# seokjuchung/point-cloud-cnn-segmentation

Measured on AMD Instinct MI355X. Metric: M voxels/sec fwd+bwd, 128^3 grid batch=4 (points/s of the PointNet training step: forward + weighted CE + backward + Adam), higher is better.
Workload: dtype bf16; 1 GPU; PointNetSegmentation train step, 4 scenes x 128^3 points per GPU, C=2; global_batch=4, parallelism=dp1

## Files before the change

point-cloud-cnn-segmentation_amd/csrc/fused_bwd.hip:

```cpp
#include "kernel_prims.h"

namespace {

constexpr int THREADS = 512;
constexpr int COUT = 512, CIN = 64, MS = 64;
constexpr int WT_ROWB = COUT * 2;
constexpr int DY_ROWB = COUT * 2 + 32;
constexpr int X_ROWB = CIN * 2 + 32;
constexpr int OFF_DY = CIN * WT_ROWB;
constexpr int OFF_X = OFF_DY + MS * DY_ROWB;
constexpr int OFF_OUT = OFF_X + MS * X_ROWB;
constexpr int OUT_ROWB = CIN * 2 + 8;
constexpr int OFF_COEF = OFF_OUT + MS * OUT_ROWB;
constexpr int OFF_H = OFF_COEF + 3 * CIN * 4;
constexpr int H_ROWB = CIN * 2;
constexpr int LDS_BYTES = OFF_H + CIN * H_ROWB;
static_assert(LDS_BYTES <= 160 * 1024, "LDS budget");
constexpr int SLAB_F = COUT * CIN + CIN * CIN + CIN;
constexpr int DY_CPR = COUT / 8, DY_RP = THREADS / DY_CPR, DY_NCH = MS / DY_RP;
constexpr int X_CPR = CIN / 8, X_RP = THREADS / X_CPR;
static_assert(X_RP == MS, "one x chunk per thread");

PCS_DEV int wt_off(int c, int slot) { return c * WT_ROWB + ((slot ^ (c & 15)) << 4); }

// ... 514 lines not shown
  for (int u = 0; u < F::TPW_D; ++u)
#pragma unroll
    for (int r = 0; r < 4; ++r)
#pragma unroll
      for (int o = 1; o < 16; o <<= 1) {
        s1[u][r] += __shfl_xor(s1[u][r], o);
        s2[u][r] += __shfl_xor(s2[u][r], o);
      }
  float2 *red = reinterpret_cast<float2 *>(lds);
  if (l16 == 0) {
#pragma unroll
    for (int u = 0; u < F::TPW_D; ++u)
#pragma unroll
      for (int r = 0; r < 4; ++r) red[mb * CB + (cbd + u) * 16 + 4 * g + r] = make_float2(s1[u][r], s2[u][r]);
  }
  __syncthreads();
  for (int c = tid; c < CB; c += THREADS) {
    float t1 = 0.f, t2 = 0.f;
#pragma unroll
    for (int b = 0; b < F::NMB; ++b) { t1 += red[b * CB + c].x; t2 += red[b * CB + c].y; }
    *reinterpret_cast<float2 *>(a.stats + ((int64_t)chunk * CIN + n0 + c) * 2) =
        make_float2(t1, a.erstd[n0 + c] * (t2 - a.emean[n0 + c] * t1));
  }
}

template <int COUT, int CIN, int CB, int MS>
int launch_bn(const pcs_gemm_args &a, float *wpart, int64_t rps, hipStream_t s) {
  const int nb = (int)(a.num_scenes * a.chunks_per_scene) * (CIN / CB);
  if (a.c_mask && a.addend) return pcs_set_einval("pcs_dgrad_wgrad_bn", "mask and addend together");
  if (a.c_mask)
    hipLaunchKernelGGL((dgrad_wgrad_bn_kernel<COUT, CIN, CB, MS, true, false>), dim3(nb), dim3(THREADS), 0, s, a, wpart, rps);
  else if (a.addend) {
    if constexpr (FB<COUT, CIN, CB, MS, false, true>::FITS)
      hipLaunchKernelGGL((dgrad_wgrad_bn_kernel<COUT, CIN, CB, MS, false, true>), dim3(nb), dim3(THREADS), 0, s, a, wpart,
                         rps);
    else
      return pcs_set_einval("pcs_dgrad_wgrad_bn", "no addend variant at this shape (LDS)");
  } else
    hipLaunchKernelGGL((dgrad_wgrad_bn_kernel<COUT, CIN, CB, MS, false, false>), dim3(nb), dim3(THREADS), 0, s, a,
                       wpart, rps);
  PCS_CHECK_LAUNCH();
  return 0;
}

struct BnShape { int cout, cin, cb, ms; };
constexpr BnShape kBnShapes[] = {{64, 64, 64, 64}, {128, 64, 64, 64}};

const BnShape *bn_shape(int K, int Ncols) {
  for (const BnShape &b : kBnShapes)
    if (b.cout == K && b.cin == Ncols) return &b;
  return nullptr;
}

}

extern "C" int64_t pcs_dgrad_wgrad_bn_workspace(pcs_gemm_args *a) {
  if (!a || a->num_scenes <= 0 || a->scene_rows <= 0) return pcs_set_einval("pcs_dgrad_wgrad_bn_workspace", "bad geometry");
  if (pcs_seg4_applicable(*a)) {
    pcs_seg4_geometry(a);
    return (int64_t)a->num_scenes * a->chunks_per_scene * a->K * a->Ncols * 4;
  }
  const BnShape *sh = bn_shape(a->K, a->Ncols);
  if (a->dtype != PCS_BF16 || !sh || (a->flags & PCS_FLAG_GENERIC))
    return pcs_set_einval("pcs_dgrad_wgrad_bn_workspace",
                          "bf16 with (Cout, Cin) = K x Ncols in {64x64, 128x64} only");
  const int nblk = sh->cin / sh->cb;
  const int64_t target = sh->cout == 64 ? 512 : 256;
  int64_t sps = (target + a->num_scenes * nblk - 1) / (a->num_scenes * nblk);
  const int64_t max_sps = (a->scene_rows + 4 * sh->ms - 1) / (4 * sh->ms);
  if (sps > max_sps) sps = max_sps;
  if (sps < 1) sps = 1;
  const int64_t rps = ((a->scene_rows + sps - 1) / sps + sh->ms - 1) / sh->ms * sh->ms;
  a->chunks_per_scene = (int32_t)((a->scene_rows + rps - 1) / rps);
  return (int64_t)a->num_scenes * a->chunks_per_scene * a->K * a->Ncols * 4;
}

extern "C" int pcs_dgrad_wgrad_bn(const pcs_gemm_args *ap, float *partial, float *dW, int64_t ldw,
                                  pcs_stream_t stream) {
  if (!ap || !partial || !dW) return pcs_set_einval("pcs_dgrad_wgrad_bn", "null argument");
  pcs_gemm_args a = *ap;
  if (pcs_dgrad_wgrad_bn_workspace(&a) < 0) return PCS_EINVAL;
  if (a.chunks_per_scene != ap->chunks_per_scene)
    return pcs_set_einval("pcs_dgrad_wgrad_bn", "chunks_per_scene must come from pcs_dgrad_wgrad_bn_workspace");
  if (!a.A || !a.A2 || !a.pa || !a.pb || !a.pc || !a.W || !a.C || !a.Yp || !a.es || !a.et || !a.emean ||
      !a.erstd || !a.stats)
    return pcs_set_einval("pcs_dgrad_wgrad_bn", "missing operand (A, A2, pa, pb, pc, W, C, Yp, es, et, emean, "
                                                "erstd, stats)");
  if (a.scene_rows * a.num_scenes >= (int64_t)1 << 31) return pcs_set_einval("pcs_dgrad_wgrad_bn", "M must be < 2^31");
  if (pcs_seg4_applicable(a)) {
    const int rc = pcs_seg4_launch(a, partial, reinterpret_cast<hipStream_t>(stream));
    if (rc) return rc;
    const int nslab = (int)(a.num_scenes * a.chunks_per_scene);
    return pcs_reduce_partials(partial, nslab, (int64_t)a.K * a.Ncols, 1.0f, dW, ldw ? ldw : a.Ncols, a.Ncols, stream);
  }
  const BnShape *sh = bn_shape(a.K, a.Ncols);
  const int64_t rps = ((a.scene_rows + a.chunks_per_scene - 1) / a.chunks_per_scene + sh->ms - 1) / sh->ms * sh->ms;
  hipStream_t s = reinterpret_cast<hipStream_t>(stream);
  int rc;
  if (a.K == 64) rc = launch_bn<64, 64, 64, 64>(a, partial, rps, s);
  else rc = launch_bn<128, 64, 64, 64>(a, partial, rps, s);
  if (rc) return rc;
  const int nslab = (int)(a.num_scenes * a.chunks_per_scene);
  return pcs_reduce_partials(partial, nslab, (int64_t)a.K * a.Ncols, 1.0f, dW, ldw ? ldw : a.Ncols, a.Ncols, stream);
}
```

point-cloud-cnn-segmentation_amd/engine.py:

```python
from __future__ import annotations

import ctypes as ct
from dataclasses import dataclass, field

import torch

from . import _lib as L

BN_EPS = 1e-5
MAX_INPUT_DIM = 8
MAX_CLASSES = 256
BN_MOMENTUM = 0.1
DROPOUT_P = 0.3

CONVS = [
    ("conv1", None, 64, "bn1"),
    ("conv2", 64, 64, "bn2"),
    ("conv3", 64, 64, "bn3"),
    ("conv4", 64, 128, "bn4"),
    ("conv5", 128, 1024, "bn5"),
    ("global_feat", 1024, 1024, "bn_global"),
    ("seg_conv1", 1088, 512, "bn_seg1"),
    ("seg_conv2", 512, 256, "bn_seg2"),
    ("seg_conv3", 256, 128, "bn_seg3"),
# ... 20 lines not shown


def flat_layout(num_classes: int, input_dim: int = 4):
    reg = dict(param_layout(num_classes, input_dim))
    names = [f"{bn}.{w}" for bn, _ in BNS for w in ("weight", "bias")]
    for conv in _EARLY_CONVS + ("global_feat",) + _SEG:
        names += [f"{conv}.weight", f"{conv}.bias"]
    return [(n, reg[n]) for n in names]


def flat_offsets(num_classes: int, input_dim: int = 4):
    offs, off = {}, 0
    for n, shape in flat_layout(num_classes, input_dim):
        offs[n] = off
        off += int(torch.Size(shape).numel())
    return offs, off


def bucket_ranges(num_classes: int, input_dim: int = 4):
    offs, total = flat_offsets(num_classes, input_dim)
    return {"seg": (offs["seg_conv1.weight"], total + FLAT_EXTRA),
            "global": (offs["global_feat.weight"], offs["seg_conv1.weight"]),
            "tail": (0, offs["global_feat.weight"])}


def check_dims(num_classes: int, input_dim: int):
    if not 1 <= int(input_dim) <= MAX_INPUT_DIM:
        raise ValueError(f"pcs_amd supports input_dim 1..{MAX_INPUT_DIM} (the reference's points carry "
                         f"4: x, y, z, e); got {input_dim}")
    if not 1 <= int(num_classes) <= MAX_CLASSES:
        raise ValueError(f"pcs_amd supports 1..{MAX_CLASSES} classes (seg_conv4 + CE head kernel); "
                         f"got {num_classes}")


def _dt(dtype: str):
    if dtype == "fp32":
        return L.F32, torch.float32
    if dtype in ("bf16", "fp8"):
        return L.BF16, torch.bfloat16
    raise ValueError(f"compute dtype must be 'fp32', 'bf16' or 'fp8', got {dtype!r}")


@dataclass(frozen=True)
class Paths:
    flags: int
    bf16: bool
    wide_fast: bool
    glds: bool
    fp8: bool
    fused12: bool
    trunk32: bool
    gram4_stats: bool
    draw_beside_gram: bool


def resolve_paths(dtype: str, flags: int = 0, eval_trunk: str = "fp32", fused_seg12: bool = True,
                  draw_beside_gram: bool = True, dropout_draw: str = "paired", *, train: bool, masks_given: bool) -> Paths:
    bf16 = dtype in ("bf16", "fp8")
    wide_fast = bf16 and not (flags & L.FLAG_GENERIC)
    return Paths(flags=flags, bf16=bf16, wide_fast=wide_fast, glds=wide_fast and not (flags & L.FLAG_NO_GLDS),
                 fp8=dtype == "fp8", fused12=bool(train and wide_fast and fused_seg12),
                 trunk32=not train and bf16 and eval_trunk == "fp32", gram4_stats=bool(train and bf16),
                 draw_beside_gram=bool(train and not masks_given and wide_fast and draw_beside_gram
                                       and dropout_draw != "independent"))


@dataclass
class BNCoef:
    mean: torch.Tensor
    rstd: torch.Tensor
    scale: torch.Tensor
    shift: torch.Tensor
    scene_sum: torch.Tensor

    def bnrelu(self):
        return dict(pa=self.scale, pb=self.shift)


@dataclass
class Saved:
    B: int
    N: int
    train: bool
    paths: Paths = None
    ys: dict = field(default_factory=dict)
    bn: dict = field(default_factory=dict)
    masks: tuple = (None, None)
    g: torch.Tensor = None
    am: torch.Tensor = None
    ysel: torch.Tensor = None
    x: torch.Tensor = None
    logits: torch.Tensor = None
    head: dict = None
    wc: dict = None
    gram4: tuple = None
    gram2: object = None
    a5_colsum: torch.Tensor = None
    gram5: tuple = None
    wg_eff: torch.Tensor = None
    sbias_s1: torch.Tensor = None
    mask_ready: object = None


def _f32(dev, *shape):
    return torch.empty(*shape, dtype=torch.float32, device=dev)


def _struct(cls, **members):
    a = cls()
    for k, v in members.items():
        setattr(a, k, L.ptr(v) if torch.is_tensor(v) else v)
    return a


class _Bwd:

    def __init__(self, gflat, offsets, bufA):
        self.gflat, self.offsets = gflat, offsets
        self.coefs = {}
        self.bufA = bufA
        self.bufB = None
        self.keep = []
        self.st = None
        self.keep_scale = 1.0 / (1.0 - DROPOUT_P)

    def G(self, name):
        return self.gflat[self.offsets[name]:]


class Engine:

    def __init__(self, num_classes: int, dtype: str = "fp32", input_dim: int = 4, eval_trunk: str = "fp32"):
        check_dims(num_classes, input_dim)
        if eval_trunk not in ("fp32", "bf16"):
            raise ValueError(f"eval_trunk must be 'fp32' or 'bf16', got {eval_trunk!r}")
        self.input_dim = input_dim
        self.C = num_classes
        self.dtype = dtype
        self.dt, self.tdt = _dt(dtype)
        self.fp8 = dtype == "fp8"
        self.a5_dt = L.FP8 if self.fp8 else self.dt
        self.eval_trunk = eval_trunk
        self.layout = param_layout(num_classes, input_dim)
        self.numel = {n: int(torch.Size(s).numel()) for n, s in self.layout}
        self.offsets, self.total_params = flat_offsets(num_classes, input_dim)
        self.buckets = bucket_ranges(num_classes, input_dim)
        self._geo = {}
        self._side = {}
        self.flags = 0
        self.timing = None
        self.timing_tags = None
        self.record_pool_rows = False
        self.last_pool_rows = None
        self.pool_rows_override = None
        self.capture = None
        self.perturb = None
        self.fused_seg12 = True
        self.draw_beside_gram = True
        self.dropout_draw = "paired"
        L.load()

    def _launch(self, tag, name, *args):
        if self.timing is None or tag is None or (self.timing_tags is not None and tag not in self.timing_tags):
            return L.call(name, *args)
        st, en = torch.cuda.Event(enable_timing=True), torch.cuda.Event(enable_timing=True)
        st.record()
        r = L.call(name, *args)
        en.record()
        self.timing.setdefault(tag, []).append((st, en))
        return r

    def _dims(self, sv):
        return sv.B, sv.N, sv.B * sv.N, sv.x.device, L.stream_ptr()

    def _side_stream(self, dev):
        st = self._side.get(dev)
        if st is None:
            st = self._side.setdefault(dev, torch.cuda.Stream(device=dev))
        return st

    @staticmethod
    def _gemm_args(B, N, K, ncols, dtype, pro=L.PRO_RAW, epi=L.EPI_FWD, cps=0, flags=0, **members):
        return _struct(L.GemmArgs, num_scenes=B, scene_rows=N, K=K, Ncols=ncols, dtype=dtype, prologue=pro,
                       epilogue=epi, chunks_per_scene=cps, flags=flags, **members)

    def geometry(self, B, N, K, ncols, pro=L.PRO_BNRELU, epi=L.EPI_FWD, dtype=None, flags=None):
        dtype = self.dt if dtype is None else dtype
        flags = self.flags if flags is None else flags
        key = (B, N, K, ncols, pro, epi, flags, dtype)
        if key not in self._geo:
            a = self._gemm_args(B, N, K, ncols, dtype, pro, epi, 0, flags)
            rpc = L.workspace("pcs_gemm_geometry", a)
            self._geo[key] = (a.chunks_per_scene, rpc)
        return self._geo[key]

    def _empty(self, *shape, dtype=None, device):
        return torch.empty(*shape, dtype=dtype or self.tdt, device=device)

    def cast_weights(self, P):
        dev = P["conv2.weight"].device
        wc = {}
        s = L.stream_ptr()
        for conv, cin, cout, _ in CONVS:
            if conv in ("conv1", "seg_conv4"):
                continue
            W = P[f"{conv}.weight"]
            rows, ld = W.shape[0], W.shape[1]
            cols = 64 if conv == "seg_conv1" else ld
            Wc = self._empty(rows, cols, device=dev)
            WcT = self._empty(cols, rows, device=dev)
# ... 37 lines not shown
        self._launch(tag, "pcs_gemm", a, L.stream_ptr())

    def _wgrad_args(self, sv, cout, cin, dy_mode, x_mode, dW, ldw=0, x_keep_scale=1.0, **members):
        return _struct(L.WgradArgs, num_scenes=sv.B, scene_rows=sv.N, Cout=cout, Cin=cin, dtype=self.dt, dy_mode=dy_mode,
                       x_mode=x_mode, x_keep_scale=x_keep_scale, dW=dW, ldw=ldw, flags=sv.paths.flags, **members)

    def _wgrad(self, sv, cout, cin, dy_mode, x_mode, dW, conv1=False, tag=None, **kw):
        a = self._wgrad_args(sv, cout, cin, dy_mode, x_mode, dW, **kw)
        if conv1:
            a.splits_per_scene = max(1, min((1024 + sv.B - 1) // sv.B, (sv.N + 255) // 256))
            nbytes = sv.B * a.splits_per_scene * cout * cin * 4
        else:
            nbytes = L.workspace("pcs_wgrad_workspace", a)
        ws = _f32(dW.device, max(nbytes // 4, 1))
        a.partial = ws.data_ptr()
        self._launch(tag, "pcs_conv1_wgrad" if conv1 else "pcs_wgrad", a, L.stream_ptr())
        return ws

    def _rounded(self, W):
        if self.dt == L.F32:
            return W
        out = torch.empty_like(W)
        L.call("pcs_round_weight", W, W.numel(), self.dt, out, L.stream_ptr())
        return out

    def _gram(self, Y, s_, t_, B, N, C, tag=None):
        dev = Y.device
        G, S = _f32(dev, C, C), _f32(dev, C)
        sps = ct.c_int32(0)
        nbytes = L.workspace("pcs_gram_workspace", B, N, C, self.dt, ct.byref(sps))
        ws = _f32(dev, max(nbytes // 4, 1))
        self._launch(tag, "pcs_gram", Y, s_, t_, B, N, C, self.dt, sps.value, ws, G, S, L.stream_ptr())
        return G, S, ws

    def _gram_raw(self, a5, G, beside=None):
        M = a5.shape[0]
        nbytes = L.workspace("pcs_gram_raw_workspace", M, 1024)
        ws = _f32(a5.device, nbytes // 4)
        if beside is not None:
            beside()
        self._launch("wgrad:global_feat", "pcs_gram_raw", a5, M, 1024, self.a5_dt, ws, nbytes, G, L.stream_ptr())
        return ws

    def forward(self, P, bufs, x, *, train, masks=None, seed=0, head_mode=L.HEAD_FWD,
                labels=None, class_weight=None, wsum=None, want_logits=True, saved=None):
        if not x.is_cuda:
            raise RuntimeError("pcs_amd runs on a HIP device only (no CPU fallback)")
        B, N, D = x.shape
        if D != self.input_dim:
            raise ValueError(f"expected x of shape (B, N, {self.input_dim}), got {tuple(x.shape)}")
        x = x.contiguous().float()
        sv = Saved(B=B, N=N, train=train) if saved is None else saved
        sv.B, sv.N, sv.train, sv.x = B, N, train, x
        sv.gram4 = None
        sv.paths = pt = resolve_paths(self.dtype, self.flags, self.eval_trunk, self.fused_seg12, self.draw_beside_gram,
                                      self.dropout_draw, train=train, masks_given=masks is not None)
        live = {}
        if train and masks is None and not pt.draw_beside_gram:
            self._draw_masks(sv, seed)
        sv.wc = self.cast_weights(P)
        self._trunk(P, bufs, sv)
        self._conv5(P, bufs, sv, live)
        self._global_feat(P, bufs, sv, live, seed)
        self._seg(P, bufs, sv, live, masks)
        sv.logits = _f32(x.device, B, N, self.C) if want_logits else None
        if head_mode == L.HEAD_CE:
            sv.head = self._head(P, sv, L.HEAD_CE, labels=labels, class_weight=class_weight, wsum=wsum)
        else:
            self._head(P, sv, L.HEAD_FWD)
        return sv

    def _draw_masks(self, sv, seed, max_wg=0):
        _, _, M, dev, _ = self._dims(sv)
        sv.masks = m1, m2 = tuple(torch.empty(M, w, dtype=torch.uint8, device=dev) for w in (64, 32))
        side = self._side_stream(dev)
        side.wait_stream(torch.cuda.current_stream(dev))
        with torch.cuda.stream(side):
            ss = L.stream_ptr()
            for i, (m, width) in enumerate(((m1, 512), (m2, 256))):
                if self.dropout_draw == "independent":
                    L.call("pcs_dropout_bits_independent", seed, i, M, width, DROPOUT_P, m, ss)
                else:
                    L.call("pcs_dropout_bits_bounded", seed, i, M, width, DROPOUT_P, m, max_wg, ss)
            sv.mask_ready = torch.cuda.Event()
            sv.mask_ready.record(side)
        m1.record_stream(side)
        m2.record_stream(side)

    def _stats_buf(self, sv, K, ncols):
        cps, rpc = self.geometry(sv.B, sv.N, K, ncols, flags=sv.paths.flags)
        return _f32(sv.x.device, sv.B * cps, ncols, 2), cps, rpc

    def _bridge(self, sv, conv, bn, K, split):
        _, _, M, dev, s = self._dims(sv)
        out = self._empty(M, 2 * K if split else K, device=dev)
        c = sv.bn[bn]
        L.call("pcs_bnrelu_bf16", sv.ys[conv], M, K, c.scale, c.shift, int(split), out, s)
        return out

    def _layer(self, P, bufs, sv, conv, src, offset=None, A_raw=None, K=None, **kw):
        M, dev = sv.B * sv.N, sv.x.device
        cin, ncols, bnname = _LAYERS[conv]
        K = K or cin
        st, cps, rpc = self._stats_buf(sv, K, ncols) if sv.train else (None, 0, 0)
        f32 = kw.get("dtype") == L.F32
        y = self._empty(M, ncols, device=dev, dtype=torch.float32 if f32 else None)
        W = P[f"{conv}.weight"] if f32 else sv.wc[conv][0]
        pro, A = L.PRO_RAW, A_raw
        if A_raw is None:
# ... 102 lines not shown
        sv.bn["bn_global"] = cg = self._bn_finalize(P, bufs, sv, "bn_global", live["stats"], 1024, cps_st, rpc_st,
                                                    P["global_feat.bias"])
        sv.g = _f32(dev, B, 1024)
        sv.am = torch.empty(B, 1024, dtype=torch.int32, device=dev)
        sv.ysel = _f32(dev, B, 1024)
        L.call("pcs_pool_finalize", pool, B, N, 1024, cps_g, cg.scale, cg.shift, sv.g, sv.am, sv.ysel, s)
        if self.record_pool_rows:
            self.last_pool_rows = sv.am.clone()
        if self.pool_rows_override is not None:
            sv.am.copy_(self.pool_rows_override)

    def _masks(self, sv, masks):
        _, _, M, dev, _ = self._dims(sv)
        m1 = m2 = None
        if sv.train and masks is not None:
            m1, m2 = masks
            if any(tuple(m.shape) != (M, w) or m.dtype != torch.uint8 or m.device != dev for m, w in ((m1, 64), (m2, 32))):
                raise ValueError(f"dropout masks must be uint8 [{M}, 64] and [{M}, 32] on {dev}, got "
                                 f"{tuple(m1.shape)} {m1.dtype} and {tuple(m2.shape)} {m2.dtype}")
            m1, m2 = m1.contiguous(), m2.contiguous()
        elif sv.train:
            m1, m2 = sv.masks
            torch.cuda.current_stream(dev).wait_event(sv.mask_ready)
        sv.masks = (m1, m2)
        return m1, m2, 1.0 / (1.0 - DROPOUT_P) if sv.train else 1.0

    def _seg(self, P, bufs, sv, live, masks):
        B, _, _, dev, s = self._dims(sv)
        pt = sv.paths
        sbias = _f32(dev, B, 512)
        live["soff"] = soff = _f32(dev, 512)
        Ws1 = P["seg_conv1.weight"]
        L.call("pcs_scene_gemv", sv.g, B, 1024, Ws1, Ws1.shape[1], 64, P["seg_conv1.bias"], 512, sbias, soff, s)
        sv.sbias_s1 = sbias
        if not pt.fused12:
            self._layer(P, bufs, sv, "seg_conv1", "conv2", soff, K=64, scene_bias=sbias,
                        A_raw=self._bridge(sv, "conv2", "bn2", 64, False) if pt.trunk32 else None)
        m1, m2, keep = self._masks(sv, masks)
        if pt.fused12:
            self._seg12(P, bufs, sv, sv.wc, sbias, soff, m1, keep)
        else:
            self._layer(P, bufs, sv, "seg_conv2", "seg_conv1", a_mask=m1, a_keep_scale=keep)
        self._layer(P, bufs, sv, "seg_conv3", "seg_conv2", a_mask=m2, a_keep_scale=keep)

    def _seg12(self, P, bufs, sv, wc, sbias, soff, m1, keep):
        B, N, M, dev, s = self._dims(sv)
        c2 = sv.bn["bn2"]
        rec = 64 * 64 + 64
        cps3 = sv.gram2.shape[0] // B
        per_scene = _f32(dev, B, rec)
        L.call("pcs_reduce_partials_grouped", sv.gram2, B, cps3, rec, 1.0, per_scene, s)
        tot = _f32(dev, rec)
        L.call("pcs_reduce_partials", per_scene, B, rec, 1.0, tot, 1, rec, s)
        G2 = tot[:64 * 64]
        Sb = per_scene[:, 64 * 64:].contiguous()
        Ws1 = P["seg_conv1.weight"]
        Ws1_r = self._rounded(Ws1)
        st1 = _f32(dev, B, 512, 2)
        L.call("pcs_bn_stats_gram_sbias", G2, Sb, B, N, Ws1_r, Ws1.shape[1], 64, 512, sbias, st1, s)
        sv.bn["bn_seg1"] = c1 = self._bn_finalize(P, bufs, sv, "bn_seg1", st1, 512, 1, N, soff)
        y1, y2 = self._empty(M, 512, device=dev), self._empty(M, 256, device=dev)
        a = _struct(L.Seg12Args, num_scenes=B, scene_rows=N, y2=sv.ys["conv2"], s2=c2.scale, t2=c2.shift,
                    W1=wc["seg_conv1"][0], sbias=sbias, Y1=y1, s1=c1.scale, t1=c1.shift, keep1=m1, keep_scale=keep,
                    W2=wc["seg_conv2"][0], Y2=y2)
        rpc, cps = L.workspace("pcs_fwd_seg12_geometry", a), a.chunks_per_scene
        st2 = _f32(dev, B * cps, 256, 2)
        a.stats = L.ptr(st2)
        self._launch("fwd:seg_conv1+2", "pcs_fwd_seg12", a, s)
        sv.ys["seg_conv1"], sv.ys["seg_conv2"] = y1, y2
        sv.bn["bn_seg2"] = self._bn_finalize(P, bufs, sv, "bn_seg2", st2, 256, cps, rpc, P["seg_conv2.bias"])

    def _head(self, P, sv, mode, labels=None, class_weight=None, wsum=None, dlogits=None):
        B, N, _, dev, s = self._dims(sv)
        c3 = sv.bn["bn_seg3"]
        ha = _struct(L.HeadArgs, num_scenes=B, scene_rows=N, Cin=128, num_classes=self.C, dtype=self.dt, mode=mode,
                     Y=sv.ys["seg_conv3"], s=c3.scale, t=c3.shift, W=P["seg_conv4.weight"], bias=P["seg_conv4.bias"],
                     logits=sv.logits if mode != L.HEAD_BWD else None)
        hb = None
        if mode != L.HEAD_FWD:
            L.workspace("pcs_head_geometry", ha)
            nch = B * ha.chunks_per_scene
            hb = dict(dZ=torch.empty(B * N * 1024, dtype=self.tdt, device=dev), stats=_f32(dev, nch, 128, 2),
                      wpartial=_f32(dev, nch, self.C * 129), loss_partial=_f32(dev, nch), cps=ha.chunks_per_scene,
                      nch=nch)
            ha.dZ, ha.stats = L.ptr(hb["dZ"]), L.ptr(hb["stats"])
            ha.wpartial, ha.loss_partial = L.ptr(hb["wpartial"]), L.ptr(hb["loss_partial"])
            ha.mean, ha.rstd = L.ptr(c3.mean), L.ptr(c3.rstd)
        if mode == L.HEAD_CE:
            ha.labels, ha.class_weight, ha.wsum = L.ptr(labels), L.ptr(class_weight), L.ptr(wsum)
        if mode == L.HEAD_BWD:
            dl = dlogits.reshape(B * N, self.C) if dlogits.dim() == 3 else dlogits
            if dl.dtype != torch.float32:
                dl = dl.float()
            ha.dlogits = L.ptr(dl)
            ha.dl_stride_row, ha.dl_stride_col = dl.stride(0), dl.stride(1)
            hb["dl"] = dl
        self._launch(f"head:{mode}", "pcs_head", ha, s)
        return hb

    def backward(self, P, sv, gflat, dlogits=None, on_bucket=None):
        bucket = on_bucket or (lambda name: None)
        if not sv.train:
            raise RuntimeError("backward needs a train-mode forward (BatchNorm batch statistics)")
        hb = self._head(P, sv, L.HEAD_BWD, dlogits=dlogits) if dlogits is not None else sv.head
        bw = _Bwd(gflat, self.offsets, hb["dZ"])
        scene_s1 = self._bwd_seg32(P, sv, bw, hb)
        sp = self._bwd_pool(P, sv, bw, scene_s1)
        dA2 = self._bwd_seg1_local(P, sv, bw)
        bucket("seg")
        Wg_r, st5, cps5 = self._bwd_global_dgrad(P, sv, bw, sp)
        self._bwd_global_wgrad(P, sv, bw, sp, Wg_r)
        bucket("global")
        self._bwd_conv5(P, sv, bw, st5, cps5)
        self._bwd_trunk(P, sv, bw, dA2)
        bucket("tail")
        return hb

    def _bn_bwd(self, P, sv, bw, bnname, conv, stats, cps, scene_s1=None):
        B, N, _, dev, s = self._dims(sv)
        fc = sv.bn[bnname]
        C = fc.mean.shape[0]
        al, be, ga = (_f32(dev, C) for _ in range(3))
        L.call("pcs_bn_bwd_finalize", stats, B, N, C, cps, fc.mean, fc.rstd, P[f"{bnname}.weight"], fc.scene_sum, al,
               be, ga, bw.G(f"{bnname}.weight"), bw.G(f"{bnname}.bias"), bw.G(f"{conv}.bias"), scene_s1, s)
        bw.coefs[bnname] = (al, be, ga)

    def _wgrad_bn(self, sv, bw, conv, dz, prev, x_mask=None, cin=None, ldw=0):
        al, be, ga = bw.coefs[_LAYERS[conv][2]]
        pc = sv.bn[_LAYERS[prev][2]]
        bw.keep.append(self._wgrad(
            sv, _LAYERS[conv][1], cin or _LAYERS[conv][0], L.PRO_BWD, L.PRO_BNRELU, bw.G(f"{conv}.weight"), ldw=ldw,
            tag=f"wgrad:{conv}", dZ=dz, Y=sv.ys[conv], alpha=al, beta=be, gamma=ga, X=sv.ys[prev], s=pc.scale,
            t=pc.shift, x_mask=x_mask, x_keep_scale=bw.keep_scale if x_mask is not None else 1.0))

    def _bwd_layer(self, P, sv, bw, conv, dz, prev, out, c_mask=None, addend=None, per_scene=False):
        B, N, _, dev, s = self._dims(sv)
        pt, WT = sv.paths, sv.wc[conv][1]
        cin, cout, bn = _LAYERS[conv]
        al, be, ga = bw.coefs[bn]
        pc = sv.bn[_LAYERS[prev][2]]
        f = dict(A2=sv.ys[conv], pa=al, pb=be, pc=ga, Yp=sv.ys[prev], es=pc.scale, et=pc.shift, emean=pc.mean,
                 erstd=pc.rstd, c_mask=c_mask, c_keep_scale=bw.keep_scale if c_mask is not None else 1.0, addend=addend)
        nbytes = -1
        if pt.wide_fast:
            a = self._gemm_args(B, N, cout, cin, self.dt, L.PRO_BWD, L.EPI_DGRAD, 0, pt.flags, A=dz, W=WT, C=out,
                                a_keep_scale=1.0, **f)
            nbytes = L.load().pcs_dgrad_wgrad_bn_workspace(ct.byref(a))
        if nbytes > 0:
            cps = a.chunks_per_scene
            st = _f32(dev, B * cps, cin, 2)
            ws = _f32(dev, nbytes // 4)
            a.stats = L.ptr(st)
            self._launch(f"dgrad+wgrad:{conv}", "pcs_dgrad_wgrad_bn", a, ws, bw.G(f"{conv}.weight"), 0, s)
            bw.keep.append(ws)
        else:
            cps, _ = self.geometry(B, N, cout, cin, L.PRO_BWD, L.EPI_DGRAD, flags=pt.flags)
            st = _f32(dev, B * cps, cin, 2)
            self._gemm(sv, cout, cin, L.PRO_BWD, L.EPI_DGRAD, dz, WT, out, stats=st, tag=f"dgrad:{conv}", **f)
            self._wgrad_bn(sv, bw, conv, dz, prev, x_mask=c_mask)
        bw.st = st
        scene_s1 = _f32(dev, B, pc.mean.shape[0]) if per_scene else None
        self._bn_bwd(P, sv, bw, _LAYERS[prev][2], prev, st, cps, scene_s1)
        return scene_s1

    def _bwd_seg32(self, P, sv, bw, hb):
        _, _, M, dev, s = self._dims(sv)
        m1, m2 = sv.masks
        L.call("pcs_reduce_partials", hb["wpartial"], hb["nch"], self.C * 129, 1.0, bw.G("seg_conv4.weight"),
               self.C * 129, self.C * 129, s)
        self._bn_bwd(P, sv, bw, "bn_seg3", "seg_conv3", hb["stats"], hb["cps"])
        bw.bufB = torch.empty(M * 1024, dtype=self.tdt, device=dev)
        self._bwd_layer(P, sv, bw, "seg_conv3", bw.bufA, "seg_conv2", bw.bufB, c_mask=m2)
        return self._bwd_layer(P, sv, bw, "seg_conv2", bw.bufB, "seg_conv1", bw.bufA, c_mask=m1, per_scene=True)

    def _bwd_pool(self, P, sv, bw, scene_s1):
        B, N, _, dev, s = self._dims(sv)
        a1, b1, g1 = bw.coefs["bn_seg1"]
        cg = sv.bn["bn_global"]
        bw.coefs["bn_global"] = ag, bg, gg = tuple(_f32(dev, 1024) for _ in range(3))
        sp = _f32(dev, B, 1024)
        csum = _f32(dev, B, 512)
        Ws1 = P["seg_conv1.weight"]
        pa = _struct(L.PoolBwdArgs, num_scenes=B, scene_rows=N, Cs=512, Cg=1024, col_off=64, s1_alpha=a1, s1_beta=b1,
                     s1_gamma=g1, s1_scene_s1=scene_s1, s1_scene_sum=sv.bn["bn_seg1"].scene_sum, W_s1=Ws1,
                     ldw=Ws1.shape[1], g=sv.g, ysel=sv.ysel, g_mean=cg.mean, g_rstd=cg.rstd,
                     g_gamma=P["bn_global.weight"], g_scene_sum=cg.scene_sum, dW_s1_global=bw.G("seg_conv1.weight"),
                     csum=csum, alpha=ag, beta_c=bg, gamma_c=gg, dgamma=bw.G("bn_global.weight"),
                     dbeta=bw.G("bn_global.bias"), dbias=bw.G("global_feat.bias"), sp=sp)
        L.call("pcs_pool_bwd", pa, s)
        bw.keep.append(csum)
        return sp

    def _bwd_seg1_local(self, P, sv, bw):
        B, N, M, dev, s = self._dims(sv)
        a1, b1, g1 = bw.coefs["bn_seg1"]
        dz_s1, ys, Ws1 = bw.bufA, sv.ys, P["seg_conv1.weight"]
        dA2 = torch.empty(M, 64, dtype=self.tdt, device=dev)
        if not sv.paths.wide_fast:
            self._gemm(sv, 512, 64, L.PRO_BWD, L.EPI_RAW, dz_s1, sv.wc["seg_conv1"][1], dA2,
                       A2=ys["seg_conv1"], pa=a1, pb=b1, pc=g1, tag="dgrad:seg_conv1")
            self._wgrad_bn(sv, bw, "seg_conv1", dz_s1, "conv2", cin=64, ldw=Ws1.shape[1])
            return dA2
        p2 = sv.bn["bn2"]
        Ws1_r = self._rounded(Ws1)
        WaT, Hs1 = self._empty(64, 512, device=dev), self._empty(64, 64, device=dev)
        L.call("pcs_bn_fold", Ws1_r, 512, 64, Ws1.shape[1], a1, b1, g1, self.dt, WaT, None, Hs1, s)
        fa = self._wgrad_args(sv, 512, 64, L.PRO_RAW, L.PRO_BNRELU, bw.G("seg_conv1.weight"), ldw=Ws1.shape[1],
                              dZ=dz_s1, alpha=a1, beta=b1, gamma=g1, X=ys["conv2"], s=p2.scale, t=p2.shift)
# ... 103 lines not shown
```

Baseline: 110.8 M points/s.

## Fold BN backward into conv3 dgrad/wgrad, reusing forward Gram to skip Y reread

Adds a folded-BN variant of the fused dgrad+wgrad kernel for conv3. It precomputes a folded weight WaT, a bias vector and a Gram-correction matrix H, so BN backward becomes a linear map of dZ plus the input activation X. This drops the read of the conv output Y (A2). Folded weights are split into bf16 hi/lo pairs to keep precision, at the cost of twice the MFMA work and more LDS. The weight gradient is assembled from reduced partials and the forward-pass Gram total, adding an assemble kernel and a reduction in exchange for less memory traffic.

```diff
diff --git a/point-cloud-cnn-segmentation_amd/csrc/fused_bwd.hip b/point-cloud-cnn-segmentation_amd/csrc/fused_bwd.hip
--- a/point-cloud-cnn-segmentation_amd/csrc/fused_bwd.hip
+++ b/point-cloud-cnn-segmentation_amd/csrc/fused_bwd.hip
@@ -590,10 +590,27 @@
   return nullptr;
 }
 
+int32_t bn_chunks(const pcs_gemm_args &a, const BnShape &sh, int64_t target) {
+  const int nblk = sh.cin / sh.cb;
+  int64_t sps = (target + a.num_scenes * nblk - 1) / (a.num_scenes * nblk);
+  const int64_t max_sps = (a.scene_rows + 4 * sh.ms - 1) / (4 * sh.ms);
+  if (sps > max_sps) sps = max_sps;
+  if (sps < 1) sps = 1;
+  const int64_t rps = ((a.scene_rows + sps - 1) / sps + sh.ms - 1) / sh.ms * sh.ms;
+  return (int32_t)((a.scene_rows + rps - 1) / rps);
+}
+
+bool bnf_selected(const pcs_gemm_args &a) {
+  return a.prologue == PCS_PRO_RAW && !pcs_seg4_applicable(a) && bn_shape(a.K, a.Ncols);
+}
+int64_t bnf_workspace(pcs_gemm_args *a);
+int bnf_run(const pcs_gemm_args *ap, float *workspace, float *dW, int64_t ldw, pcs_stream_t stream);
+
 }
 
 extern "C" int64_t pcs_dgrad_wgrad_bn_workspace(pcs_gemm_args *a) {
   if (!a || a->num_scenes <= 0 || a->scene_rows <= 0) return pcs_set_einval("pcs_dgrad_wgrad_bn_workspace", "bad geometry");
+  if (bnf_selected(*a)) return bnf_workspace(a);
   if (pcs_seg4_applicable(*a)) {
     pcs_seg4_geometry(a);
     return (int64_t)a->num_scenes * a->chunks_per_scene * a->K * a->Ncols * 4;
@@ -602,20 +619,14 @@
   if (a->dtype != PCS_BF16 || !sh || (a->flags & PCS_FLAG_GENERIC))
     return pcs_set_einval("pcs_dgrad_wgrad_bn_workspace",
                           "bf16 with (Cout, Cin) = K x Ncols in {64x64, 128x64} only");
-  const int nblk = sh->cin / sh->cb;
-  const int64_t target = sh->cout == 64 ? 512 : 256;
-  int64_t sps = (target + a->num_scenes * nblk - 1) / (a->num_scenes * nblk);
-  const int64_t max_sps = (a->scene_rows + 4 * sh->ms - 1) / (4 * sh->ms);
-  if (sps > max_sps) sps = max_sps;
-  if (sps < 1) sps = 1;
-  const int64_t rps = ((a->scene_rows + sps - 1) / sps + sh->ms - 1) / sh->ms * sh->ms;
-  a->chunks_per_scene = (int32_t)((a->scene_rows + rps - 1) / rps);
+  a->chunks_per_scene = bn_chunks(*a, *sh, sh->cout == 64 ? 512 : 256);
   return (int64_t)a->num_scenes * a->chunks_per_scene * a->K * a->Ncols * 4;
 }
 
 extern "C" int pcs_dgrad_wgrad_bn(const pcs_gemm_args *ap, float *partial, float *dW, int64_t ldw,
                                   pcs_stream_t stream) {
   if (!ap || !partial || !dW) return pcs_set_einval("pcs_dgrad_wgrad_bn", "null argument");
+  if (bnf_selected(*ap)) return bnf_run(ap, partial, dW, ldw, stream);
   pcs_gemm_args a = *ap;
   if (pcs_dgrad_wgrad_bn_workspace(&a) < 0) return PCS_EINVAL;
   if (a.chunks_per_scene != ap->chunks_per_scene)
@@ -641,3 +652,374 @@
   const int nslab = (int)(a.num_scenes * a.chunks_per_scene);
   return pcs_reduce_partials(partial, nslab, (int64_t)a.K * a.Ncols, 1.0f, dW, ldw ? ldw : a.Ncols, a.Ncols, stream);
 }
+
+namespace {
+
+template <int COUT, bool ADD> struct FF {
+  static constexpr int CIN = 64, MS = 64;
+  static constexpr int WT_ROWB = COUT * 2, WSW = COUT >= 128 ? 15 : 7;
+  static constexpr int DY_ROWB = COUT * 2 + 32, X_ROWB = CIN * 2 + 32;
+  static constexpr int YP_ROWB = CIN * 2 + 16, OUT_ROWB = CIN * 2 + 8, H_ROWB = CIN * 2;
+  static constexpr int OFF_DY = CIN * WT_ROWB;
+  static constexpr int OFF_X = OFF_DY + MS * DY_ROWB;
+  static constexpr int OFF_YP = OFF_X + MS * X_ROWB;
+  static constexpr int OFF_AD = OFF_YP + MS * YP_ROWB;
+  static constexpr int OFF_OUT = OFF_AD + (ADD ? MS * YP_ROWB : 0);
+  static constexpr int OFF_COEF = OFF_OUT + MS * OUT_ROWB;
+  static constexpr int OFF_H = OFF_COEF + 3 * CIN * 4;
+  static constexpr int OFF_HL = OFF_H + CIN * H_ROWB;
+  static constexpr int OFF_WL = OFF_HL + CIN * H_ROWB;
+  static constexpr int BYTES = OFF_WL + CIN * WT_ROWB;
+  static constexpr int CBW = COUT / 32;
+  static constexpr int NCH_D = MS * COUT / 8 / THREADS;
+  static_assert(MS * CIN / 8 == THREADS, "one Yp chunk per thread");
+  static_assert(4 * CIN * 8 <= OFF_DY, "end-of-pass S1 / S2 reduction area");
+};
+
+constexpr int bnf_slab(int cout, bool withg = true) { return cout * 64 + (withg ? 64 * 64 + 64 : 0); }
+
+template <int COUT, bool ADD, bool WITHG>
+__global__ __launch_bounds__(THREADS) __attribute__((amdgpu_waves_per_eu(COUT == 64 ? 4 : 1, 8))) void dgrad_wgrad_bnf_kernel(
+    pcs_gemm_args a, float *__restrict__ wpart, int64_t rows_per_split) {
+  typedef FF<COUT, ADD> F;
+  constexpr int CIN = F::CIN, MS = F::MS;
+  static_assert((COUT == 64 ? 2 : 1) * F::BYTES <= 160 * 1024, "LDS budget");
+  __shared__ __attribute__((aligned(16))) char lds[F::BYTES];
+  const int tid = threadIdx.x, lane = tid & 63, wid = tid >> 6;
+  const int chunk = xcd_remap(blockIdx.x, gridDim.x);
+  const int sps = a.chunks_per_scene;
+  const int scene = chunk / sps, sis = chunk % sps;
+  const int64_t N = a.scene_rows;
+  const int64_t lo = (int64_t)sis * rows_per_split;
+  const int64_t hi = pcs_min64(lo + rows_per_split, N);
+  const int64_t sbase = (int64_t)scene * N;
+  const bf16_t *__restrict__ dZ = reinterpret_cast<const bf16_t *>(a.A);
+  const bf16_t *__restrict__ Ypg = reinterpret_cast<const bf16_t *>(a.Yp);
+  const bf16_t *__restrict__ Adg = reinterpret_cast<const bf16_t *>(a.addend);
+  const float *__restrict__ Wt = reinterpret_cast<const float *>(a.W);
+  const float *__restrict__ Hg = reinterpret_cast<const float *>(a.W2);
+  bf16_t *__restrict__ Cg = reinterpret_cast<bf16_t *>(a.C);
+
+  auto split_to_lds = [&](const float *src, char *hi_dst, char *lo_dst) {
+    float v[8], h[8];
+    *reinterpret_cast<float4 *>(v) = *reinterpret_cast<const float4 *>(src);
+    *reinterpret_cast<float4 *>(v + 4) = *reinterpret_cast<const float4 *>(src + 4);
+    const u32x4 hi = pack_chunk(v);
+    unpack_chunk(hi, h);
+#pragma unroll
+    for (int e = 0; e < 8; ++e) v[e] -= h[e];
+    *reinterpret_cast<u32x4 *>(hi_dst) = hi;
+    *reinterpret_cast<u32x4 *>(lo_dst) = pack_chunk(v);
+  };
+  for (int i = tid; i < CIN * COUT / 8; i += THREADS) {
+    const int c = i / (COUT / 8), slot = i % (COUT / 8);
+    const int off = c * F::WT_ROWB + ((slot ^ (c & F::WSW)) << 4);
+    split_to_lds(Wt + (int64_t)c * COUT + slot * 8, lds + off, lds + F::OFF_WL + off);
+  }
+  {
+    const int c = tid / (CIN / 8), slot = tid % (CIN / 8);
+    const int off = c * F::H_ROWB + ((slot ^ (c & 7)) << 4);
+    split_to_lds(Hg + (int64_t)c * CIN + slot * 8, lds + F::OFF_H + off, lds + F::OFF_HL + off);
+  }
+  float *cf = reinterpret_cast<float *>(lds + F::OFF_COEF);
+  if (tid < CIN) { cf[tid] = a.es[tid]; cf[CIN + tid] = a.et[tid]; cf[2 * CIN + tid] = a.bias[tid]; }
+  __syncthreads();
+
+  const int pr = tid / (CIN / 8), pc = tid % (CIN / 8);
+  u32x4 rz[F::NCH_D], rp, rd;
+  auto load_step = [&](int64_t m0) {
+#pragma unroll
+    for (int i = 0; i < F::NCH_D; ++i) {
+      const int q = tid + THREADS * i, rl = q / (COUT / 8), cc = q % (COUT / 8);
+      rz[i] = *reinterpret_cast<const u32x4 *>(dZ + (sbase + pcs_min64(m0 + rl, hi - 1)) * COUT + cc * 8);
+    }
+    const int64_t off = (sbase + pcs_min64(m0 + pr, hi - 1)) * CIN + pc * 8;
+    rp = *reinterpret_cast<const u32x4 *>(Ypg + off);
+    if constexpr (ADD) rd = *reinterpret_cast<const u32x4 *>(Adg + off);
+  };
+  auto store_step = [&](int64_t m0) {
+#pragma unroll
+    for (int i = 0; i < F::NCH_D; ++i) {
+      const int q = tid + THREADS * i, rl = q / (COUT / 8), cc = q % (COUT / 8);
+      const u32x4 out = m0 + rl >= hi ? mk_u32x4(0, 0, 0, 0) : rz[i];
+      *reinterpret_cast<u32x4 *>(lds + F::OFF_DY + prow(rl) * F::DY_ROWB + cc * 16) = out;
+    }
+    float s8[8], t8[8], v[8];
+    lds_vec8(cf + pc * 8, s8); lds_vec8(cf + CIN + pc * 8, t8);
+    unpack_chunk(rp, v);
+#pragma unroll
+    for (int e = 0; e < 8; ++e) v[e] = relu(fmaf(v[e], s8[e], t8[e]));
+    u32x4 out = pack_chunk(v);
+    if (m0 + pr >= hi) out = mk_u32x4(0, 0, 0, 0);
+    *reinterpret_cast<u32x4 *>(lds + F::OFF_X + prow(pr) * F::X_ROWB + pc * 16) = out;
+    *reinterpret_cast<u32x4 *>(lds + F::OFF_YP + pr * F::YP_ROWB + pc * 16) = rp;
+    if constexpr (ADD) *reinterpret_cast<u32x4 *>(lds + F::OFF_AD + pr * F::YP_ROWB + pc * 16) = rd;
+  };
+
+  f32x4 accw[F::CBW];
+#pragma unroll
+  for (int u = 0; u < F::CBW; ++u) accw[u] = f32x4{0.f, 0.f, 0.f, 0.f};
+  f32x4 accg[2] = {f32x4{0.f, 0.f, 0.f, 0.f}, f32x4{0.f, 0.f, 0.f, 0.f}};
+  float xs = 0.f;
+  float s1[2][4], s2[2][4];
+#pragma unroll
+  for (int u = 0; u < 2; ++u)
+#pragma unroll
+    for (int r = 0; r < 4; ++r) { s1[u][r] = 0.f; s2[u][r] = 0.f; }
+
+  const int nsteps = (int)((hi - lo + MS - 1) / MS);
+  if (nsteps > 0) {
+    load_step(lo);
+    store_step(lo);
+    __builtin_amdgcn_sched_barrier(0);
+    load_step(lo + MS);
+  }
+  __syncthreads();
+
+  const int g = lane >> 4, l16 = lane & 15;
+  const int mb = wid >> 1, cbd = 2 * (wid & 1);
+  const int ob0 = wid * F::CBW / 4, cbw = wid * F::CBW % 4;
+  const char *tDY = lds + F::OFF_DY, *tX = lds + F::OFF_X;
+  const int ml = mb * 16 + l16;
+  constexpr bool ROOMY = COUT != 64;
+  auto h_frag = [&](int off_img, int kk, int u) {
+    const int c = (cbd + u) * 16 + l16;
+    return *reinterpret_cast<const bf16x8 *>(lds + off_img + c * F::H_ROWB + (((4 * kk + g) ^ (c & 7)) << 4));
+  };
+  bf16x8 hreg[ROOMY ? 2 : 1][2][2];
+  if constexpr (ROOMY) {
+#pragma unroll
+    for (int kk = 0; kk < 2; ++kk)
+#pragma unroll
+      for (int u = 0; u < 2; ++u) { hreg[0][kk][u] = h_frag(F::OFF_H, kk, u); hreg[1][kk][u] = h_frag(F::OFF_HL, kk, u); }
+  }
+  for (int st = 0; st < nsteps; ++st) {
+    const int64_t m0 = lo + (int64_t)st * MS;
+    f32x4 accd[2];
+#pragma unroll
+    for (int u = 0; u < 2; ++u) accd[u] = *reinterpret_cast<const f32x4 *>(cf + 2 * CIN + (cbd + u) * 16 + 4 * g);
+    if constexpr (ROOMY) {
+      f32x4 accl[2] = {f32x4{0.f, 0.f, 0.f, 0.f}, f32x4{0.f, 0.f, 0.f, 0.f}};
+#pragma unroll
+      for (int kk = 0; kk < COUT / 32; ++kk) {
+        const int slot = 4 * kk + g;
+        const bf16x8 yf = *reinterpret_cast<const bf16x8 *>(tDY + prow(ml) * F::DY_ROWB + slot * 16);
+#pragma unroll
+        for (int u = 0; u < 2; ++u) {
+          const int c = (cbd + u) * 16 + l16;
+          const int off = c * F::WT_ROWB + ((slot ^ (c & F::WSW)) << 4);
+          const bf16x8 wf = *reinterpret_cast<const bf16x8 *>(lds + off);
+          const bf16x8 wl = *reinterpret_cast<const bf16x8 *>(lds + F::OFF_WL + off);
+          accd[u] = __builtin_amdgcn_mfma_f32_16x16x32_bf16(wf, yf, accd[u], 0, 0, 0);
+          accl[u] = __builtin_amdgcn_mfma_f32_16x16x32_bf16(wl, yf, accl[u], 0, 0, 0);
+        }
+      }
+#pragma unroll
+      for (int kk = 0; kk < CIN / 32; ++kk) {
+        const bf16x8 xf = *reinterpret_cast<const bf16x8 *>(tX + prow(ml) * F::X_ROWB + (4 * kk + g) * 16);
+#pragma unroll
+        for (int u = 0; u < 2; ++u) {
+          accd[u] = __builtin_amdgcn_mfma_f32_16x16x32_bf16(hreg[0][kk][u], xf, accd[u], 0, 0, 0);
+          accl[u] = __builtin_amdgcn_mfma_f32_16x16x32_bf16(hreg[1][kk][u], xf, accl[u], 0, 0, 0);
+        }
+      }
+#pragma unroll
+      for (int u = 0; u < 2; ++u) accd[u] += accl[u];
+    } else {
+#pragma unroll
+      for (int kk = 0; kk < COUT / 32; ++kk) {
+        const int slot = 4 * kk + g;
+        const bf16x8 yf = *reinterpret_cast<const bf16x8 *>(tDY + prow(ml) * F::DY_ROWB + slot * 16);
+#pragma unroll
+        for (int u = 0; u < 2; ++u) {
+          const int c = (cbd + u) * 16 + l16;
+          const int off = c * F::WT_ROWB + ((slot ^ (c & F::WSW)) << 4);
+          const bf16x8 wf = *reinterpret_cast<const bf16x8 *>(lds + off);
+          const bf16x8 wl = *reinterpret_cast<const bf16x8 *>(lds + F::OFF_WL + off);
+          accd[u] = __builtin_amdgcn_mfma_f32_16x16x32_bf16(wf, yf, accd[u], 0, 0, 0);
+          accd[u] = __builtin_amdgcn_mfma_f32_16x16x32_bf16(wl, yf, accd[u], 0, 0, 0);
+        }
+      }
+#pragma unroll
+      for (int kk = 0; kk < CIN / 32; ++kk) {
+        const int slot = 4 * kk + g;
+        const bf16x8 xf = *reinterpret_cast<const bf16x8 *>(tX + prow(ml) * F::X_ROWB + slot * 16);
+#pragma unroll
+        for (int u = 0; u < 2; ++u) {
+          const int c = (cbd + u) * 16 + l16;
+          const int off = c * F::H_ROWB + ((slot ^ (c & 7)) << 4);
+          const bf16x8 hf = *reinterpret_cast<const bf16x8 *>(lds + F::OFF_H + off);
+          const bf16x8 hl = *reinterpret_cast<const bf16x8 *>(lds + F::OFF_HL + off);
+          accd[u] = __builtin_amdgcn_mfma_f32_16x16x32_bf16(hf, xf, accd[u], 0, 0, 0);
+          accd[u] = __builtin_amdgcn_mfma_f32_16x16x32_bf16(hl, xf, accd[u], 0, 0, 0);
+        }
+      }
+    }
+#pragma unroll
+    for (int kk = 0; kk < MS / 32; ++kk) {
+      const int q = (lane >> 2) & 3, p = lane & 3;
+      const int r0 = prow(32 * kk + 8 * g + q), r1 = prow(32 * kk + 8 * g + 4 + q);
+      const bf16x8 yf = tr_read(tDY, r0, r1, F::DY_ROWB, ob0 * 16 + 4 * p);
+      bf16x8 xi;
+      if constexpr (WITHG) {
+        xi = tr_read(tX, r0, r1, F::X_ROWB, mb * 16 + 4 * p);
+        const u32x4 xu = __builtin_bit_cast(u32x4, xi);
+        xs += ((bf_lo(xu.x) + bf_hi(xu.x)) + (bf_lo(xu.y) + bf_hi(xu.y))) +
+              ((bf_lo(xu.z) + bf_hi(xu.z)) + (bf_lo(xu.w) + bf_hi(xu.w)));
+      }
+#pragma unroll
+      for (int u = 0; u < F::CBW; ++u) {
+        const bf16x8 xf = tr_read(tX, r0, r1, F::X_ROWB, (cbw + u) * 16 + 4 * p);
+        accw[u] = __builtin_amdgcn_mfma_f32_16x16x32_bf16(xf, yf, accw[u], 0, 0, 0);
+        if constexpr (F::CBW == 2 && WITHG) accg[u] = __builtin_amdgcn_mfma_f32_16x16x32_bf16(xf, xi, accg[u], 0, 0, 0);
+      }
+      if constexpr (F::CBW != 2 && WITHG) {
+#pragma unroll
+        for (int u = 0; u < 2; ++u) {
+          const bf16x8 xj = tr_read(tX, r0, r1, F::X_ROWB, (cbd + u) * 16 + 4 * p);
+          accg[u] = __builtin_amdgcn_mfma_f32_16x16x32_bf16(xj, xi, accg[u], 0, 0, 0);
+        }
+      }
+    }
+    const bool live = m0 + ml < hi;
+#pragma unroll
+    for (int u = 0; u < 2; ++u) {
+      const int c = (cbd + u) * 16 + 4 * g;
+      const uint2 yp = *reinterpret_cast<const uint2 *>(lds + F::OFF_YP + ml * F::YP_ROWB + c * 2);
+      const float y[4] = {bf_lo(yp.x), bf_hi(yp.x), bf_lo(yp.y), bf_hi(yp.y)};
+      float v[4] = {accd[u][0], accd[u][1], accd[u][2], accd[u][3]};
+      if constexpr (ADD) {
+        const uint2 ad = *reinterpret_cast<const uint2 *>(lds + F::OFF_AD + ml * F::YP_ROWB + c * 2);
+        v[0] += bf_lo(ad.x); v[1] += bf_hi(ad.x); v[2] += bf_lo(ad.y); v[3] += bf_hi(ad.y);
+      }
+#pragma unroll
+      for (int r = 0; r < 4; ++r) {
+        const float dz = (live && fmaf(y[r], cf[c + r], cf[CIN + c + r]) > 0.f) ? v[r] : 0.f;
+        v[r] = dz;
+        s1[u][r] += dz;
+        s2[u][r] = fmaf(dz, y[r], s2[u][r]);
+      }
+      *reinterpret_cast<uint2 *>(lds + F::OFF_OUT + ml * F::OUT_ROWB + c * 2) =
+          make_uint2(pack2bf(v[0], v[1]), pack2bf(v[2], v[3]));
+    }
+    lds_barrier();
+    if (m0 + pr < hi)
+      st16(Cg + (sbase + m0 + pr) * CIN + pc * 8,
+           *reinterpret_cast<const u32x4 *>(lds + F::OFF_OUT + pr * F::OUT_ROWB + pc * 16));
+    if (st + 1 < nsteps) {
+      store_step(m0 + MS);
+      __builtin_amdgcn_sched_barrier(0);
+      load_step(m0 + 2 * MS);
+    }
+    lds_barrier();
+  }
+
+  float *out = wpart + (int64_t)chunk * bnf_slab(COUT, WITHG);
+#pragma unroll
+  for (int u = 0; u < F::CBW; ++u)
+    *reinterpret_cast<float4 *>(out + (ob0 * 16 + l16) * CIN + (cbw + u) * 16 + 4 * g) =
+        make_float4(accw[u][0], accw[u][1], accw[u][2], accw[u][3]);
+  if constexpr (WITHG) {
+#pragma unroll
+    for (int u = 0; u < 2; ++u)
+      *reinterpret_cast<float4 *>(out + COUT * CIN + (mb * 16 + l16) * CIN + (cbd + u) * 16 + 4 * g) =
+          make_float4(accg[u][0], accg[u][1], accg[u][2], accg[u][3]);
+  }
+
+  if constexpr (WITHG) {
+    xs += __shfl_xor(xs, 16);
+    xs += __shfl_xor(xs, 32);
+    if (!(wid & 1) && g == 0) out[COUT * CIN + CIN * CIN + mb * 16 + l16] = xs;
+  }
+
+#pragma unroll
+  for (int u = 0; u < 2; ++u)
+#pragma unroll
+    for (int r = 0; r < 4; ++r)
+#pragma unroll
+      for (int o = 1; o < 16; o <<= 1) {
+        s1[u][r] += __shfl_xor(s1[u][r], o);
+        s2[u][r] += __shfl_xor(s2[u][r], o);
+      }
+  float2 *red = reinterpret_cast<float2 *>(lds);
+  if (l16 == 0) {
+#pragma unroll
+    for (int u = 0; u < 2; ++u)
+#pragma unroll
+      for (int r = 0; r < 4; ++r) red[mb * CIN + (cbd + u) * 16 + 4 * g + r] = make_float2(s1[u][r], s2[u][r]);
+  }
+  __syncthreads();
+  if (tid < CIN) {
+    float t1 = 0.f, t2 = 0.f;
+#pragma unroll
+    for (int b = 0; b < 4; ++b) { t1 += red[b * CIN + tid].x; t2 += red[b * CIN + tid].y; }
+    *reinterpret_cast<float2 *>(a.stats + ((int64_t)chunk * CIN + tid) * 2) =
+        make_float2(t1, a.erstd[tid] * (t2 - a.emean[tid] * t1));
+  }
+}
+
+__global__ __launch_bounds__(64) void bnf_assemble_kernel(const float *__restrict__ red, const float *__restrict__ GS,
+                                                          const float *__restrict__ W, int64_t ldwin,
+                                                          const float *__restrict__ alpha, const float *__restrict__ beta,
+                                                          const float *__restrict__ gamma, float *__restrict__ dW,
+                                                          int64_t ldo) {
+  constexpr int CIN = 64;
+  __shared__ float wk[CIN];
+  const int o = blockIdx.x, k = threadIdx.x;
+  wk[k] = W[(int64_t)o * ldwin + k];
+  __syncthreads();
+  const float *G = GS, *S = G + CIN * CIN;
+  double wg = 0.0;
+  for (int j = 0; j < CIN; ++j) wg += (double)wk[j] * (double)G[j * CIN + k];
+  const double v = (double)alpha[o] * (double)red[o * CIN + k] + ((double)beta[o] * (double)S[k] + (double)gamma[o] * wg);
+  dW[(int64_t)o * ldo + k] = (float)v;
+}
+
+int64_t bnf_workspace(pcs_gemm_args *a) {
+  const BnShape *sh = bn_shape(a->K, a->Ncols);
+  if (a->dtype != PCS_BF16 || !sh || (a->flags & PCS_FLAG_GENERIC) || a->c_mask)
+    return pcs_set_einval("pcs_dgrad_wgrad_bn_workspace",
+                          "folded form (PCS_PRO_RAW): bf16 with (Cout, Cin) = K x Ncols in {64x64, 128x64}, no c_mask only");
+  a->chunks_per_scene = bn_chunks(*a, *sh, sh->cout == 64 ? 512 : 256);
+  return ((int64_t)a->num_scenes * a->chunks_per_scene + 1) * bnf_slab(a->K) * 4;
+}
+
+template <int COUT>
+void launch_bnf(const pcs_gemm_args &a, bool withg, int nslab, float *ws, int64_t rps, hipStream_t s) {
+  const dim3 grid(nslab), block(THREADS);
+  if (a.addend && withg) hipLaunchKernelGGL((dgrad_wgrad_bnf_kernel<COUT, true, true>), grid, block, 0, s, a, ws, rps);
+  else if (a.addend) hipLaunchKernelGGL((dgrad_wgrad_bnf_kernel<COUT, true, false>), grid, block, 0, s, a, ws, rps);
+  else if (withg) hipLaunchKernelGGL((dgrad_wgrad_bnf_kernel<COUT, false, true>), grid, block, 0, s, a, ws, rps);
+  else hipLaunchKernelGGL((dgrad_wgrad_bnf_kernel<COUT, false, false>), grid, block, 0, s, a, ws, rps);
+}
+
+int bnf_run(const pcs_gemm_args *ap, float *workspace, float *dW, int64_t ldw, pcs_stream_t stream) {
+  pcs_gemm_args a = *ap;
+  if (bnf_workspace(&a) < 0) return PCS_EINVAL;
+  if (a.chunks_per_scene != ap->chunks_per_scene)
+    return pcs_set_einval("pcs_dgrad_wgrad_bn", "chunks_per_scene must come from pcs_dgrad_wgrad_bn_workspace");
+  const float *W = a.pool_w, *GS = a.gram;
+  const int64_t ldw_in = a.pool_ldw;
+  if (!a.A || !a.pa || !a.pb || !a.pc || !a.W || !a.W2 || !a.bias || !a.C || !a.Yp || !a.es || !a.et || !a.emean ||
+      !a.erstd || !a.stats || !W || ldw_in < a.Ncols || (ldw && ldw < a.Ncols))
+    return pcs_set_einval("pcs_dgrad_wgrad_bn", "folded form: missing operand (A, pa, pb, pc, W, W2, bias, C, Yp, es, "
+                                                "et, emean, erstd, stats, pool_w; pool_ldw, ldw >= Cin)");
+  if (a.scene_rows * a.num_scenes >= (int64_t)1 << 31) return pcs_set_einval("pcs_dgrad_wgrad_bn", "M must be < 2^31");
+  const int MS = 64;
+  const int64_t rps = ((a.scene_rows + a.chunks_per_scene - 1) / a.chunks_per_scene + MS - 1) / MS * MS;
+  const int nslab = (int)(a.num_scenes * a.chunks_per_scene);
+  hipStream_t s = reinterpret_cast<hipStream_t>(stream);
+  const bool withg = GS == nullptr;
+  if (a.K == 64) launch_bnf<64>(a, withg, nslab, workspace, rps, s);
+  else launch_bnf<128>(a, withg, nslab, workspace, rps, s);
+  PCS_CHECK_LAUNCH();
+  const int64_t slab = bnf_slab(a.K, withg);
+  float *red = workspace + (int64_t)nslab * slab;
+  if (int rc = pcs_reduce_partials(workspace, nslab, slab, 1.0f, red, slab, slab, stream)) return rc;
+  hipLaunchKernelGGL(bnf_assemble_kernel, dim3(a.K), dim3(64), 0, s, red, withg ? red + a.K * 64 : GS, W, ldw_in,
+                     a.pa, a.pb, a.pc, dW, ldw ? ldw : a.Ncols);
+  PCS_CHECK_LAUNCH();
+  return 0;
+}
+
+}
diff --git a/point-cloud-cnn-segmentation_amd/engine.py b/point-cloud-cnn-segmentation_amd/engine.py
--- a/point-cloud-cnn-segmentation_amd/engine.py
+++ b/point-cloud-cnn-segmentation_amd/engine.py
@@ -96,17 +96,19 @@
     trunk32: bool
     gram4_stats: bool
     draw_beside_gram: bool
+    folded_trunk: bool = True
 
 
 def resolve_paths(dtype: str, flags: int = 0, eval_trunk: str = "fp32", fused_seg12: bool = True,
-                  draw_beside_gram: bool = True, dropout_draw: str = "paired", *, train: bool, masks_given: bool) -> Paths:
+                  draw_beside_gram: bool = True, dropout_draw: str = "paired", *, train: bool, masks_given: bool,
+                  folded_trunk: bool = True) -> Paths:
     bf16 = dtype in ("bf16", "fp8")
     wide_fast = bf16 and not (flags & L.FLAG_GENERIC)
     return Paths(flags=flags, bf16=bf16, wide_fast=wide_fast, glds=wide_fast and not (flags & L.FLAG_NO_GLDS),
                  fp8=dtype == "fp8", fused12=bool(train and wide_fast and fused_seg12),
                  trunk32=not train and bf16 and eval_trunk == "fp32", gram4_stats=bool(train and bf16),
                  draw_beside_gram=bool(train and not masks_given and wide_fast and draw_beside_gram
-                                       and dropout_draw != "independent"))
+                                       and dropout_draw != "independent"), folded_trunk=bool(folded_trunk))
 
 
 @dataclass
@@ -139,6 +141,7 @@
     wc: dict = None
     gram4: tuple = None
     gram2: object = None
+    gram2_total: torch.Tensor = None
     a5_colsum: torch.Tensor = None
     gram5: tuple = None
     wg_eff: torch.Tensor = None
@@ -200,6 +203,7 @@
         self.capture = None
         self.perturb = None
         self.fused_seg12 = True
+        self.folded_trunk = True
         self.draw_beside_gram = True
         self.dropout_draw = "paired"
         L.load()
@@ -343,9 +347,10 @@
         x = x.contiguous().float()
         sv = Saved(B=B, N=N, train=train) if saved is None else saved
         sv.B, sv.N, sv.train, sv.x = B, N, train, x
-        sv.gram4 = None
+        sv.gram4 = sv.gram2_total = None
         sv.paths = pt = resolve_paths(self.dtype, self.flags, self.eval_trunk, self.fused_seg12, self.draw_beside_gram,
-                                      self.dropout_draw, train=train, masks_given=masks is not None)
+                                      self.dropout_draw, train=train, masks_given=masks is not None,
+                                      folded_trunk=self.folded_trunk)
         live = {}
         if train and masks is None and not pt.draw_beside_gram:
             self._draw_masks(sv, seed)
@@ -554,6 +559,7 @@
         L.call("pcs_reduce_partials_grouped", sv.gram2, B, cps3, rec, 1.0, per_scene, s)
         tot = _f32(dev, rec)
         L.call("pcs_reduce_partials", per_scene, B, rec, 1.0, tot, 1, rec, s)
+        sv.gram2_total = tot
         G2 = tot[:64 * 64]
         Sb = per_scene[:, 64 * 64:].contiguous()
         Ws1 = P["seg_conv1.weight"]
@@ -644,18 +650,34 @@
         f = dict(A2=sv.ys[conv], pa=al, pb=be, pc=ga, Yp=sv.ys[prev], es=pc.scale, et=pc.shift, emean=pc.mean,
                  erstd=pc.rstd, c_mask=c_mask, c_keep_scale=bw.keep_scale if c_mask is not None else 1.0, addend=addend)
         nbytes = -1
-        if pt.wide_fast:
-            a = self._gemm_args(B, N, cout, cin, self.dt, L.PRO_BWD, L.EPI_DGRAD, 0, pt.flags, A=dz, W=WT, C=out,
-                                a_keep_scale=1.0, **f)
-            nbytes = L.load().pcs_dgrad_wgrad_bn_workspace(ct.byref(a))
-        if nbytes > 0:
+        if pt.wide_fast and pt.folded_trunk and conv == "conv3" and sv.gram2_total is not None:
+            W = P[f"{conv}.weight"]
+            W_r = self._rounded(W)
+            WaT, cv, H = _f32(dev, cin, cout), _f32(dev, cin), _f32(dev, cin, cin)
+            L.call("pcs_bn_fold", W_r, cout, cin, W.shape[1], al, be, ga, L.F32, WaT, cv, H, s)
+            del f["A2"]
+            a = self._gemm_args(B, N, cout, cin, self.dt, L.PRO_RAW, L.EPI_DGRAD, 0, pt.flags, A=dz, W=WaT, W2=H,
+                                bias=cv, C=out, a_keep_scale=1.0, pool_w=W_r, pool_ldw=W.shape[1],
+                                gram=sv.gram2_total, **f)
+            nbytes = L.workspace("pcs_dgrad_wgrad_bn_workspace", a)
             cps = a.chunks_per_scene
             st = _f32(dev, B * cps, cin, 2)
             ws = _f32(dev, nbytes // 4)
             a.stats = L.ptr(st)
             self._launch(f"dgrad+wgrad:{conv}", "pcs_dgrad_wgrad_bn", a, ws, bw.G(f"{conv}.weight"), 0, s)
-            bw.keep.append(ws)
-        else:
+            bw.keep.append((ws, W_r, WaT, cv, H))
+        elif pt.wide_fast:
+            a = self._gemm_args(B, N, cout, cin, self.dt, L.PRO_BWD, L.EPI_DGRAD, 0, pt.flags, A=dz, W=WT, C=out,
+                                a_keep_scale=1.0, **f)
+            nbytes = L.load().pcs_dgrad_wgrad_bn_workspace(ct.byref(a))
+            if nbytes > 0:
+                cps = a.chunks_per_scene
+                st = _f32(dev, B * cps, cin, 2)
+                ws = _f32(dev, nbytes // 4)
+                a.stats = L.ptr(st)
+                self._launch(f"dgrad+wgrad:{conv}", "pcs_dgrad_wgrad_bn", a, ws, bw.G(f"{conv}.weight"), 0, s)
+                bw.keep.append(ws)
+        if nbytes <= 0:
             cps, _ = self.geometry(B, N, cout, cin, L.PRO_BWD, L.EPI_DGRAD, flags=pt.flags)
             st = _f32(dev, B * cps, cin, 2)
             self._gemm(sv, cout, cin, L.PRO_BWD, L.EPI_DGRAD, dz, WT, out, stats=st, tag=f"dgrad:{conv}", **f)
```

Result: no change. 111.3 M points/s (median of 6 runs) (+0.5%).
